# StephenTaf/Modern-Search-Engines-Project

Measured on AMD Instinct MI355X. Metric: queries/sec, two-stage retrieval top-100 (BM25 top-1000 + dense full scan + rerank/fuse), higher is better.
Workload: dtype f32 (exact f32 cosines of every returned document; candidates filtered by one pass of f16 products with a measured margin; batches <= 64 queries: f16x2-split products, |err| <= 8e-6) (dense cosine) / f64 (BM25, fuse)

## Files before the change

include/msretr.h:

```cpp
#ifndef MSRETR_H
#define MSRETR_H

#include <stdint.h>

#ifdef __cplusplus
extern "C" {
#endif

#define MSR_ABI_VERSION 15
#define MSR_DIM 768
#define MSR_MAX_K 1024
#define MSR_MAX_QUERY_TERMS 64
#define MSR_RERANK_MAX_CHUNKS 10
#define MSR_TERMSET_SPAN_DOCS 8192
#define MSR_PHRASE_MAX_TERMS 16
#define MSR_PROX_MAX_SPAN 64
#define MSR_SNIPPET_MAX_WEIGHT (1 << 20)
#define MSR_FUZZY_MAX_LEN 32
#define MSR_FUZZY_MAX_WORDS 1024
#define MSR_FUZZY_MAX_LIMIT 16
#define MSR_FUZZY_SPAN_TERMS 1024
#define MSR_FUZZY_WORD_GROUP 16
#define MSR_WILD_MAX_LEN 32
#define MSR_WILD_MAX_PATTERNS 1024
// ... 13 lines not shown

typedef struct msr_config {
    int32_t struct_size;
    int32_t device;
    int32_t dim;
    int32_t max_queries;
    int32_t max_k;
    int32_t rerank_max_docs;
    int32_t scan_layout;
    int32_t scan_variant;
    int32_t flags;
} msr_config;

#define MSR_CFG_NO_ROW_COPY 1
#define MSR_CFG_SINGLE_EMIT 2

typedef struct msr_rerank_params {
    double smoothing;
    double max_boost;
    double max_decay;
    int32_t max_chunks;
    int32_t reserved;
} msr_rerank_params;

int msr_abi_version(void);
int msr_create(const msr_config* cfg, msr_engine** out);
int msr_destroy(msr_engine* e);
const char* msr_last_error(const msr_engine* e);

int msr_bind_postings(msr_engine* e, const int64_t* term_off, int64_t n_terms, const int32_t* post_doc,
// ... 205 lines not shown
```

modern-search-engines-project_amd/_abi.py:

```python
import ctypes as C
import os

HERE = os.path.dirname(os.path.abspath(__file__))
LIB_PATH = os.path.join(HERE, "csrc", "libmsretr.so")

MSR_ABI_VERSION = 15
MSR_CFG_NO_ROW_COPY = 1
MSR_CFG_SINGLE_EMIT = 2
MSR_DIM = 768
MSR_MAX_K = 1024
MSR_MAX_QUERY_TERMS = 64
MSR_RERANK_MAX_CHUNKS = 10
MSR_MERGE_MAX_ENTRIES = 8192
MSR_TERMSET_SPAN_DOCS = 8192
MSR_PHRASE_MAX_TERMS = 16
MSR_PROX_MAX_SPAN = 64
MSR_SNIPPET_MAX_WEIGHT = 1 << 20
MSR_FUZZY_MAX_LEN = 32
MSR_FUZZY_MAX_WORDS = 1024
MSR_FUZZY_MAX_LIMIT = 16
MSR_FUZZY_SPAN_TERMS = 1024
MSR_FUZZY_WORD_GROUP = 16
MSR_WILD_MAX_LEN = 32
MSR_WILD_MAX_PATTERNS = 1024
# ... 146 lines not shown
```

modern-search-engines-project_amd/csrc/msr_engine.hip:

```cpp
#include <hip/hip_runtime.h>
#include <stdarg.h>
#include <stdio.h>
#include <stdlib.h>
#include <string.h>

#include <algorithm>
#include <new>
#include <vector>

#include "../../include/msretr.h"
#include "msr_devmem.h"
#include "msr_internal.h"

struct HipMem {
    static hipError_t alloc(void** p, size_t bytes) { return hipMalloc(p, bytes); }
    static void free(void* p) { (void)hipFree(p); }
};
using Group = DevGroup<HipMem>;

struct msr_engine {
    msr_config cfg;
    char err[512];
    Group mem_engine;
    Group mem_corpus;
// ... 45 lines not shown
    uint64_t* bm_win = nullptr;
    uint64_t* voc_sig = nullptr;
    int32_t* bt_top_doc = nullptr; float* bt_top_score = nullptr; int32_t* bt_top_n = nullptr;
    int32_t* bt_cand_doc = nullptr; float* bt_cand_score = nullptr; int32_t* bt_cand_chunk = nullptr;
    int32_t* bt_cand_n = nullptr;
    int32_t* tile_row = nullptr;
    int n_tiles = 0;
    bool tiles_ok = false;
    GemmF32Index gf{};
    bool gf_ok = false;
    float* gf_inv_pad = nullptr; float* gf_qn = nullptr; void* gf_fb_qimg = nullptr;
    int32_t* gf_gate = nullptr;
    void* gf_emb_tiled = nullptr;
    void* gf_emb_f16 = nullptr;
    int32_t* tile_trow = nullptr;
    void* emb_bf16 = nullptr;
    GemmIndex gemm{};
    bool gemm_ok = false;
    float* gm_qn = nullptr;
    uint32_t* bf_err = nullptr;
    float* bf_margin = nullptr;
    float* bf_ones = nullptr;
    void* bf_row_meta = nullptr;
    DenseIndex dense_bf16{};
    int n_cus = 256;
    int split_pending = 0;
    int row_copy_state = 0;
    int row_image_state = 0;
    int last_dense_width = 0;
    int last_dense_segments = 0;
// ... 52 lines not shown
    e->mem_postings.release();
}
static void drop_bf16(msr_engine* e) {
    e->dense.emb_bf16 = nullptr;
    e->dense_bf16 = DenseIndex{};
    e->gemm = GemmIndex{};
    e->gemm_ok = false;
    e->mem_bf16.release();
}
static void drop_chunks(msr_engine* e) {
    e->have_chunks = false;
    e->split_pending = 0;
    e->dense = DenseIndex{};
    e->gf = GemmF32Index{};
    e->gf_ok = e->tiles_ok = false;
    e->n_tiles = 0;
    e->row_copy_state = e->row_image_state = 0;
    drop_bf16(e);
    e->mem_chunks.release();
}

template <class T>
static int grow(msr_engine* e, Group& group, T** slot, size_t* have, size_t need, const char* what) {
    if (need <= *have && *slot) return MSR_OK;
    group.free_one(slot);
    *have = 0;
    hipError_t herr = group.alloc(slot, need);
    if (herr != hipSuccess) return fail(e, MSR_ERR_NOMEM, "%s (%zu bytes): %s", what, need, hipGetErrorString(herr));
    *have = need;
    return MSR_OK;
}
// ... 44 lines not shown
    *out = nullptr;
    if (cfg->struct_size != (int32_t)sizeof(msr_config))
        return fail(nullptr, MSR_ERR_INVALID, "msr_create: struct_size %d != %zu", cfg->struct_size, sizeof(msr_config));
    if (cfg->dim != MSR_DIM) return fail(nullptr, MSR_ERR_INVALID, "msr_create: dim must be %d", MSR_DIM);
    if (cfg->max_queries < 1 || cfg->max_queries > 4096)
        return fail(nullptr, MSR_ERR_INVALID, "msr_create: max_queries out of range [1, 4096]");
    if (cfg->max_k < 1 || cfg->max_k > MSR_MAX_K)
        return fail(nullptr, MSR_ERR_INVALID, "msr_create: max_k out of range [1, %d]", MSR_MAX_K);
    if (cfg->rerank_max_docs < 0 || cfg->rerank_max_docs > 1024)
        return fail(nullptr, MSR_ERR_INVALID, "msr_create: rerank_max_docs out of range [0, 1024]");
    if (cfg->scan_layout != 0 && cfg->scan_layout != 1)
        return fail(nullptr, MSR_ERR_INVALID, "msr_create: scan_layout must be 0 or 1");
    if (cfg->scan_variant != 0 && cfg->scan_variant != 2 && cfg->scan_variant != 7 && cfg->scan_variant != 14 &&
        cfg->scan_variant != 15)
        return fail(nullptr, MSR_ERR_INVALID, "msr_create: scan_variant must be 0, 2, 7, 14 or 15");
    if (cfg->flags & ~(int32_t)(MSR_CFG_NO_ROW_COPY | MSR_CFG_SINGLE_EMIT))
        return fail(nullptr, MSR_ERR_INVALID, "msr_create: unknown flag bits 0x%x", cfg->flags);
    int ndev = 0;
    hipError_t herr = hipGetDeviceCount(&ndev);
    if (herr != hipSuccess || ndev <= 0)
        return fail(nullptr, MSR_ERR_HIP, "msr_create: no HIP device available (%s)",
                    herr == hipSuccess ? "device count is 0" : hipGetErrorString(herr));
    if (cfg->device < 0 || cfg->device >= ndev)
        return fail(nullptr, MSR_ERR_INVALID, "msr_create: device %d out of range (have %d)", cfg->device, ndev);
    msr_engine* e = new (std::nothrow) msr_engine();
    if (!e) return fail(nullptr, MSR_ERR_NOMEM, "msr_create: out of host memory");
    e->cfg = *cfg;
    e->err[0] = 0;
    const int rc = create_scratch(e);
    if (rc) {
        fail(nullptr, rc, "msr_create: %s", e->err);
// ... 126 lines not shown
    const Bm25Index cand{term_off, post_doc, post_tf, doc_len, idf, n_terms, n_postings, n_docs, (double)avgdl, k1, b,
                         nullptr, nullptr, (int32_t)((n_docs + MSR_BM25_TILE - 1) / MSR_BM25_TILE), nullptr, nullptr, nullptr, 0};
    const int rc = build_postings(e, cand, (hipStream_t)stream);
    if (rc) drop_postings(e);
    e->have_postings = rc == MSR_OK;
    return rc;
}

struct ChunkLayout {
    std::vector<int32_t> spans, wspans, wspans12;
    int wide_ok = 1, wide_ok64 = 1;
    bool tiles_ok = true;
    std::vector<int32_t> tiles;
    std::vector<int32_t> trow;
    int64_t n_trows = 0;
};

static int chunk_layout(msr_engine* e, int n_cus, const std::vector<int32_t>& h_off, int64_t n_chunks, int64_t n_docs,
                        ChunkLayout& L) {
    if (h_off[0] != 0 || (int64_t)h_off[n_docs] != n_chunks)
        return fail(e, MSR_ERR_INVALID, "msr_bind_chunks: doc_off[0]=%d, doc_off[n_docs]=%d, n_chunks=%lld",
                    h_off[0], h_off[n_docs], (long long)n_chunks);
    for (int64_t d = 0; d < n_docs; ++d)
        if (h_off[d + 1] < h_off[d]) return fail(e, MSR_ERR_INVALID, "msr_bind_chunks: doc_off not monotone at %lld", (long long)d);
    auto make_spans = [&](int target, int64_t min_rows) {
        if ((int64_t)target * min_rows > n_chunks) target = (int)std::max<int64_t>(1, n_chunks / min_rows);
        std::vector<int32_t> sp;
        sp.push_back(0);
        for (int s = 1; s < target; ++s) {
            const int64_t want = n_chunks * s / target;
// ... 47 lines not shown
    L.tiles.push_back(0);
    for (int64_t d = 0; d < n_docs && L.tiles_ok; ++d) {
        const int32_t end = h_off[d + 1];
        if (end - h_off[d] > 256) L.tiles_ok = false;
        if (end - start > 256) { L.tiles.push_back(h_off[d]); start = h_off[d]; }
    }
    if (!L.tiles_ok) return MSR_OK;
    if (L.tiles.back() != (int32_t)n_chunks) L.tiles.push_back((int32_t)n_chunks);
    const size_t n_tiles = L.tiles.size() - 1;
    L.trow.resize(n_tiles);
    for (size_t t = 0; t < n_tiles; ++t) {
        L.trow[t] = (int32_t)L.n_trows;
        L.n_trows += (L.tiles[t + 1] - L.tiles[t] + 15) / 16 * 16;
    }
    if (L.n_trows + MSR_STREAM256_TILE_ROWS >= ((int64_t)1 << 31)) { L.trow.clear(); L.n_trows = 0; }
    return MSR_OK;
}

static int bind_chunk_tables(msr_engine* e, const float* emb, int64_t n_chunks, const int32_t* doc_off, int64_t n_docs,
                             const float* inv_norm, const ChunkLayout& L, hipStream_t st) {
    ALLOC(e, e->mem_chunks, e->chunk_doc, (size_t)n_chunks * sizeof(int32_t));
    ALLOC(e, e->mem_chunks, e->span_doc, L.spans.size() * sizeof(int32_t));
    ALLOC(e, e->mem_chunks, e->wspan_doc, L.wspans.size() * sizeof(int32_t));
    HIP_TRY(e, hipMemcpyAsync(e->span_doc, L.spans.data(), L.spans.size() * sizeof(int32_t), hipMemcpyHostToDevice, st));
    HIP_TRY(e, hipMemcpyAsync(e->wspan_doc, L.wspans.data(), L.wspans.size() * sizeof(int32_t), hipMemcpyHostToDevice, st));
    ALLOC(e, e->mem_chunks, e->wspan12_doc, L.wspans12.size() * sizeof(int32_t));
    HIP_TRY(e, hipMemcpyAsync(e->wspan12_doc, L.wspans12.data(), L.wspans12.size() * sizeof(int32_t), hipMemcpyHostToDevice, st));
    HIP_TRY(e, msr_fill_chunk_doc(doc_off, n_docs, e->chunk_doc, st));
    if (!inv_norm) {
        ALLOC(e, e->mem_chunks, e->inv_norm_own, (size_t)n_chunks * sizeof(float));
// ... 22 lines not shown
        } else {
            ALLOC(e, e->mem_chunks, e->emb_presplit, (size_t)n_chunks * MSR_DIM * sizeof(float));
            HIP_TRY(e, msr_presplit_rows(emb, n_chunks, e->emb_presplit, st));
        }
    }
    e->dense = DenseIndex{emb, doc_off, e->chunk_doc, inv_norm, e->span_doc, n_chunks, n_docs, (n_docs + 31) / 32 * 32,
                          (int)L.spans.size() - 1, e->cfg.scan_layout, e->wspan_doc, (int)L.wspans.size() - 1, e->wspan12_doc,
                          (int)L.wspans12.size() - 1, e->qimg, nullptr, e->emb_presplit, e->row_meta, L.wide_ok,
                          L.wide_ok && L.wide_ok64, nullptr, variant};
    if (L.tiles_ok) {
        ALLOC(e, e->mem_chunks, e->tile_row, L.tiles.size() * 4);
        HIP_TRY(e, hipMemcpyAsync(e->tile_row, L.tiles.data(), L.tiles.size() * 4, hipMemcpyHostToDevice, st));
        e->n_tiles = (int)L.tiles.size() - 1;
        e->tiles_ok = true;
    }
    if (!L.trow.empty()) {
        ALLOC(e, e->mem_chunks, e->tile_trow, L.trow.size() * 4);
        HIP_TRY(e, hipMemcpyAsync(e->tile_trow, L.trow.data(), L.trow.size() * 4, hipMemcpyHostToDevice, st));
    }
    HIP_TRY(e, hipStreamSynchronize(st));
    return MSR_OK;
}

static int bind_stream_pass(msr_engine* e, const ChunkLayout& L, hipStream_t st) {
    if (!(e->tiles_ok && e->dense.variant == 14 && e->n_tiles >= 64)) return MSR_OK;
    const float* emb = e->dense.emb;
    const float* inv_norm = e->dense.inv_norm;
    const int64_t n_chunks = e->dense.n_chunks;
    const int n_tiles = e->n_tiles, nw = e->n_cus * 8, stride = (n_tiles + 31) / 32 * 32;
    const int groups = std::min(8, std::max(e->cfg.max_queries, 128) / 128);
    const int GF_WV_CAP = 4096 * std::max(1, groups / 2);
    const size_t QM = (size_t)groups * 128;
    const int max_nt = std::max(1, std::min(4, groups / 2));
    GemmF32Index& g = e->gf;
    g.n_tiles = n_tiles; g.n_cus = e->n_cus; g.max_groups = groups; g.tmax_stride = stride; g.wv_cap = GF_WV_CAP; g.max_nt = max_nt;
    g.single_emit = (e->cfg.flags & MSR_CFG_SINGLE_EMIT) ? 1 : 0;
    ALLOC(e, e->mem_chunks, e->gf_inv_pad, (size_t)(n_chunks + 512) * 4);
    ALLOC(e, e->mem_chunks, g.qimg, (size_t)groups * 24 * 8192);
    ALLOC(e, e->mem_chunks, e->gf_qn, (QM + 64) * MSR_DIM * 4);
    ALLOC(e, e->mem_chunks, e->gf_fb_qimg, (QM + 63) / 64 * msr_ksplit_slice_image_bytes());
    ALLOC(e, e->mem_chunks, g.tmax_t, (size_t)n_tiles * 8 * (groups >= 2 ? 256 * max_nt : 128) * 4);
    ALLOC(e, e->mem_chunks, g.tmax, QM * stride * 4);
    ALLOC(e, e->mem_chunks, g.thr, QM * 4);
    ALLOC(e, e->mem_chunks, g.thr2, QM * 4);
    ALLOC(e, e->mem_chunks, g.flag, QM * 4);
    ALLOC(e, e->mem_chunks, g.wvbuf, (size_t)nw * GF_WV_CAP * 16);
    ALLOC(e, e->mem_chunks, g.wv_count, (size_t)nw * 4);
    ALLOC(e, e->mem_chunks, g.pairs, QM * 4096 * 8);
    ALLOC(e, e->mem_chunks, g.pair_n, QM * 4);
    ALLOC(e, e->mem_chunks, e->gf_gate, GF_GATE_BYTES);
    ALLOC(e, e->mem_chunks, g.err_max, 4);
    ALLOC(e, e->mem_chunks, g.margin, QM * 4);
    ALLOC(e, e->mem_chunks, g.cand_doc, QM * MSR_SEL_CAP * 4);
    ALLOC(e, e->mem_chunks, g.cand_score, QM * MSR_SEL_CAP * 4);
    ALLOC(e, e->mem_chunks, g.cand_chunk, QM * MSR_SEL_CAP * 4);
    ALLOC(e, e->mem_chunks, g.cand_n, QM * 4);
    g.tile_row = e->tile_row;
    g.inv_pad = e->gf_inv_pad;
    HIP_TRY(e, msr_pad_inv_norm(inv_norm, n_chunks, n_chunks + 512, e->gf_inv_pad, st));
    HIP_TRY(e, hipMemsetAsync(g.pair_n, 0, QM * 4, st));
    HIP_TRY(e, hipMemsetAsync(e->gf_gate, 0, GF_GATE_BYTES, st));
    HIP_TRY(e, hipMemsetAsync(g.cand_n, 0, QM * 4, st));
    HIP_TRY(e, msr_f16_row_error(emb, inv_norm, n_chunks, g.err_max, st));
    if (groups >= 2 && e->tile_trow) {
        const size_t copy_rows = (size_t)L.n_trows + MSR_STREAM256_TILE_ROWS;
        if ((int64_t)L.trow.back() + MSR_STREAM256_TILE_ROWS > (int64_t)copy_rows)
            return fail(e, MSR_ERR_INVALID, "msr_bind_chunks: internal: tile table exceeds the fragment-order copy");
        if (e->cfg.flags & MSR_CFG_NO_ROW_COPY) {
            e->row_copy_state = 2;
        } else if (e->mem_chunks.alloc(&e->gf_emb_tiled, copy_rows * MSR_DIM * 4) != hipSuccess) {
            (void)hipGetLastError();
            e->row_copy_state = 3;
        } else {
            HIP_TRY(e, hipMemsetAsync((char*)e->gf_emb_tiled + (size_t)L.n_trows * MSR_DIM * 4, 0,
                                      (size_t)MSR_STREAM256_TILE_ROWS * MSR_DIM * 4, st));
            HIP_TRY(e, msr_tile_rows(emb, e->tile_row, e->tile_trow, n_tiles, e->gf_emb_tiled, st));
            e->row_copy_state = 1;
        }
    }
    if (max_nt >= 2 && (e->cfg.flags & MSR_CFG_NO_ROW_COPY)) {
        e->row_image_state = 2;
    } else if (max_nt >= 2) {
        const size_t img_rows = (size_t)n_chunks + 512;
        if (e->mem_chunks.alloc(&e->gf_emb_f16, img_rows * MSR_DIM * 2) != hipSuccess) {
            (void)hipGetLastError();
            e->row_image_state = 3;
        } else {
            HIP_TRY(e, msr_f16_rows(emb, n_chunks, (int64_t)img_rows, e->gf_emb_f16, st));
            e->row_image_state = 1;
        }
    }
    g.emb_tiled = e->gf_emb_tiled;
    g.tile_trow = e->gf_emb_tiled ? e->tile_trow : nullptr;
    g.emb_f16 = e->gf_emb_f16;
    e->gf_ok = true;
    return MSR_OK;
}

extern "C" int msr_bind_chunks(msr_engine* e, const float* emb, int64_t n_chunks, const int32_t* doc_off,
                               int64_t n_docs, const float* inv_norm, void* stream) {
    if (!e) return MSR_ERR_INVALID;
    if (!emb || !doc_off || n_chunks <= 0 || n_chunks >= (1ll << 31) || n_docs <= 0 || n_docs >= (1ll << 31))
        return fail(e, MSR_ERR_INVALID, "msr_bind_chunks: bad argument");
    if (e->have_postings && e->bm25.n_docs != n_docs)
        return fail(e, MSR_ERR_INVALID, "msr_bind_chunks: n_docs %lld differs from bound postings (%lld)",
                    (long long)n_docs, (long long)e->bm25.n_docs);
    if (e->cfg.scan_layout == 1 && !inv_norm)
        return fail(e, MSR_ERR_INVALID, "msr_bind_chunks: inv_norm is required with the interleaved layout");
// ... 649 lines not shown
    HIP_TRY(e, msr_dense_scan_slices(ix, e->gf_qn, nq, (float*)e->score_rows, e->gf_fb_qimg, st));
    SelScratch sel = e->sel;
    sel.gate = e->gf_gate; sel.gate_per64 = 1;
    HIP_TRY(e, msr_select_topk(32, e->score_rows, N, e->dense.score_stride, nq, k, sel, out_doc, out_score, out_n, st));
    ix.gate = e->gf_gate; ix.gate_per64 = 1;
    if (out_chunk) HIP_TRY(e, msr_best_chunk(ix, e->gf_qn, nq, k, 0, out_doc, out_n, out_chunk, st));
    return MSR_OK;
}

static bool dense_sweep_wide(const msr_engine* e, int max_chunks_per_doc) {
    return (e->dense.variant == 2 || e->dense.variant == 14 || e->dense.variant == 15) && e->dense.layout == 0 &&
           e->dense.wide_ok && max_chunks_per_doc == 0;
}

static bool dense_stream_ok(const msr_engine* e, int k) {
    return dense_sweep_wide(e, 0) && e->gf_ok && e->dense.variant == 14 && e->gf.n_tiles >= 2 * k;
}

static int dense_stream_cap(const msr_engine* e) { return e->gf.max_groups >= 2 ? (e->gf.max_groups & ~1) * 128 : 128; }

static hipEvent_t* pass_events(msr_engine* e, int kind, hipEvent_t ev[4]) {
    if (!e->timing || e->ev_count[kind] >= msr_engine::EV_RING || e->ev_count[3] >= msr_engine::EV_RING) return nullptr;
    ev[0] = e->ev_start[3][e->ev_count[3]]; ev[1] = e->ev_stop[3][e->ev_count[3]];
    ev[2] = e->ev_start[kind][e->ev_count[kind]]; ev[3] = e->ev_stop[kind][e->ev_count[kind]];
    return ev;
}
static void pass_events_used(msr_engine* e, int kind, const hipEvent_t* ev) {
    if (ev) { e->ev_count[kind]++; e->ev_count[3]++; }
}

extern "C" int msr_dense_split_max(const msr_engine* e, int32_t k) {
// ... 585 lines not shown
```

modern-search-engines-project_amd/csrc/msr_gemm_f32.hip:

```cpp
#include <cmath>
#include <type_traits>

#include "msr_common.h"
#include "msr_internal.h"
#include "msr_frag.h"
#include "msr_gemm_dev.h"

namespace {

constexpr int GF_THREADS = 512;
constexpr int GF_KT = MSR_DIM / 32;
constexpr int GF_ROWB = MSR_DIM * 4;
constexpr int GF_PAIR_CAP = 4096;

typedef StreamArgs GemmF32Args;

__device__ __forceinline__ const char* uniform_ptr(const char* p) {
    const uint64_t u = (uint64_t)p;
    const uint32_t lo = __builtin_amdgcn_readfirstlane((uint32_t)u), hi = __builtin_amdgcn_readfirstlane((uint32_t)(u >> 32));
    return (const char*)(((uint64_t)hi << 32) | lo);
}

constexpr int GS_NB = 8;
constexpr int GS_STEP = 8192;
// ... 322 lines not shown
            return b;
        };
#pragma unroll
        for (int j = 0; j < NNI / 2; ++j) {
            const float lo = a.thr[grp * 256 + (2 * j) * 16 + li16], hi = a.thr[grp * 256 + (2 * j + 1) * 16 + li16];
            thr_h[j] = down_h(lo) | (down_h(hi) << 16);
        }
    }
    constexpr bool JOIN = BF16;
    uint32_t* tmx = (uint32_t*)(smem + G2_TMX);
    if (JOIN) tmx[tid] = 0u;
    auto flush_tmax = [&](int tile_j, int par) {
        const int ln = (int)fresh_lane();
        if (ln < 32) {
            uint32_t* slot = tmx + par * 256 + w * 32 + ln;
            a.tmax_t[(size_t)tile_j * nq_pad + grp * 256 + w * 32 + ln] = ord_val(*slot);
            *slot = 0u;
        }
    };
    float* inv_lds = (float*)(smem + 2 * G2_BLK + 1024) + w * 64;
    auto stage_b = [&](int blk, int pb) {
        const char* base = uniform_ptr(qimg + (size_t)blk * G2_BLK + (size_t)w * 8192);
#pragma unroll
        for (int i = 0; i < 8; ++i)
            __builtin_amdgcn_global_load_lds((glb_void*)(base + (uint32_t)(i * 1024 + lane * 16)),
                                             (lds_void*)(smem + pb * G2_BLK + w * 8192 + i * 1024), 16, 0, 0);
    };
    f32x4 acc[NMI][NNI];
#pragma unroll
    for (int mi = 0; mi < NMI; ++mi)
#pragma unroll
        for (int ni = 0; ni < NNI; ++ni) acc[mi][ni] = (f32x4){0.f, 0.f, 0.f, 0.f};

    auto tile_of = [&](int j) { return a.t_first + j * a.t_stride; };
    auto tile_base = [&](int row0) { return uniform_u64((uint64_t)a.E + (uint64_t)row0 * ROWB); };
    constexpr int NV = (BF16 || TILED) ? 1 : NMI;
    auto row_off = [&](int row0, int mi) -> uint32_t {
        if (TILED) return (uint32_t)(lane * 16);
        if (BF16) return (uint32_t)((WROWS * wr + li16) * ROWB + lg * 32);
        int64_t r = (int64_t)row0 + WROWS * wr + 16 * mi + li16;
        if (r > a.n_rows - 1) r = a.n_rows - 1;
        return (uint32_t)((r - row0) * ROWB + lg * 32);
    };
    int jt = gid;
    int row0 = a.tile_row[tile_of(jt)], row_end = a.tile_row[tile_of(jt) + 1];
    int jn = jt + G < a.t_count ? jt + G : jt;
    int row0n = a.tile_row[tile_of(jn)];
    uint64_t bp = tile_base(TILED ? a.tile_trow[tile_of(jt)] : row0), bn = tile_base(TILED ? a.tile_trow[tile_of(jn)] : row0n);
    uint32_t vp[NV], vn[NV];
#pragma unroll
    for (int mi = 0; mi < NV; ++mi) { vp[mi] = row_off(row0, mi); vn[mi] = row_off(row0n, mi); }

    static_assert(NMI == 2, "the wait counts below assume 4 row loads per ring slot");
    f32x4 ring[RSLOTS][NMI][2];
    auto load_rows = [&](auto slot_c, uint64_t sb, const uint32_t* v, auto off_c) {
        constexpr int slot = decltype(slot_c)::value, off = decltype(off_c)::value;
#pragma unroll
        for (int mi = 0; mi < NMI; ++mi) {
            if (TILED) {
                const uint64_t b = sb + (uint64_t)((2 * wr + mi) * ((GF_KT / KPS) * 2048) + slot * 2048);
                gload16s<0, NTL>(ring[slot][mi][0], v[0], b);
                gload16s<1024, NTL>(ring[slot][mi][1], v[0], b);
            } else {
// ... 144 lines not shown
            if (!(a.dbg & 131072))
#endif
            wg_barrier();
            pb ^= 1;
            if (JOIN && kb == 0 && it > 0) flush_tmax(jt_prev, (it - 1) & 1);
        }
        const int ln_e = (int)fresh_lane();
        const int lg_e = ln_e >> 4;
        f32x4 inv4[NMI];
        if (!BF16 || F16I) {
            if (F16I) asm volatile("s_waitcnt vmcnt(8)" ::: "memory");
            else asm volatile("s_waitcnt vmcnt(12)" ::: "memory");
#pragma unroll
            for (int mi = 0; mi < NMI; ++mi) inv4[mi] = *(const f32x4*)(inv_lds + mi * 16 + 4 * lg_e);
        }
        const int n_valid = row_end - row0;
        const int col_e = wc * 128 + (ln_e & 15);
        float thr_nx = (EMIT && !THR_REGS) ? thr_lds[col_e] : 0.f;
#ifdef MSR_DIAG
        if (a.dbg & 65536) {
#pragma unroll
            for (int ni = 0; ni < NNI; ++ni)
#pragma unroll
                for (int mi = 0; mi < NMI; ++mi) acc[mi][ni] = (f32x4){0.f, 0.f, 0.f, 0.f};
        } else
#endif
#pragma unroll
        for (int ni = 0; ni < NNI; ++ni) {
            f32x4 v[NMI];
            float cmax = NEG_INF;
            const float thr_cur = thr_nx;
// ... 29 lines not shown
                                const int pos = wave_cnt + (int)__builtin_amdgcn_mbcnt_hi((uint32_t)(hm >> 32), __builtin_amdgcn_mbcnt_lo((uint32_t)hm, 0u));
                                if (hit && pos < a.wv_cap)
                                    wvbuf[pos] = make_int4(row0 + rb + rr, q, __float_as_int(x), tile_of(jt));
                                wave_cnt += __popcll(hm);
                            }
                        }
                    }
                }
            }
            float m = cmax;
            auto s32 = __builtin_amdgcn_permlane32_swap(__float_as_uint(m), __float_as_uint(m), false, false);
            m = max2_raw(__uint_as_float(s32[0]), __uint_as_float(s32[1]));
            auto s16 = __builtin_amdgcn_permlane16_swap(__float_as_uint(m), __float_as_uint(m), false, false);
            m = max2_raw(__uint_as_float(s16[0]), __uint_as_float(s16[1]));
            if (JOIN) {
                if (lg_e == 0) atomicMax(tmx + (it & 1) * 256 + ni * 16 + col_e, ord_key(m));
            } else {
                if (lg_e == 0) a.tmax_t[((size_t)jt * 8 + w) * nq_pad + grp * 256 + ni * 16 + col_e] = m;
            }
        }
        jt_prev = jt;
        jt = jn;
        row0 = row0n;
        row_end = a.tile_row[tile_of(jt) + 1];
        jn = jt + G < a.t_count ? jt + G : jt;
        row0n = a.tile_row[tile_of(jn)];
        bp = bn; bn = tile_base(TILED ? a.tile_trow[tile_of(jn)] : row0n);
#pragma unroll
        for (int mi = 0; mi < NV; ++mi) { vp[mi] = vn[mi]; vn[mi] = row_off(row0n, mi); }
    }
    wait_vm0();
    if (JOIN) {
        wg_barrier();
        flush_tmax(jt_prev, (n_mine - 1) & 1);
    }
    if (EMIT && lane == 0) a.wv_count[blockIdx.x * 8 + w] = wave_cnt;
}

template <bool BF16, bool TOBF16 = BF16>
__global__ __launch_bounds__(256) void build_qimg2_kernel(const float* __restrict__ qn, int nq, f16x8* __restrict__ qimg) {
    const int i = blockIdx.x * 256 + threadIdx.x;
    if (i >= GF_KT * 256 * 4) return;
// ... 295 lines not shown
    if (dbg & 8388608) t1 = 2 * t1;
#endif
    if (t1 >= std::max(grid, 2 * k) && T - t1 >= grid) {
        p.n_seg = 2; p.bound[1] = (int)t1; p.bound[2] = T;
    }
    return p;
}

}

hipError_t msr_gemm_f32_pass(const GemmF32Index& g, const DenseIndex& ix, const float* qn, int nq, int k, int k_part,
                             float* out_part, hipEvent_t* ev, int* width_out, int* seg_out, hipStream_t stream) {
    const int W = nq > 128 ? 256 : 128;
    const int waves = 8;
    const int G = (nq + W - 1) / W;
    if (nq <= 0 || G * W > 128 * g.max_groups || k < 1 || g.n_tiles < 2 * k) return hipErrorInvalidValue;
    if (width_out) *width_out = W;
    hipError_t err;
    int NT0 = 1;
    if (W == 256 && (g.n_cus & 7) == 0) NT0 = std::min(std::min(G, g.max_nt), g.n_cus >> 3);
    bool image16 = W == 256 && NT0 > 1 && g.emb_f16 != nullptr;
#ifdef MSR_DIAG
    if (g_f32_dbg & (2048 | 1048576)) image16 = false;
#endif
    if (image16) build_qimg2_kernel<true, false><<<dim3((GF_KT * 256 * 4 + 255) / 256, G), 256, 0, stream>>>(qn, nq, (f16x8*)g.qimg);
    else if (W == 256) build_qimg2_kernel<false><<<dim3((GF_KT * 256 * 4 + 255) / 256, G), 256, 0, stream>>>(qn, nq, (f16x8*)g.qimg);
    else build_qimg1_kernel<<<dim3((GF_KT * 128 * 4 + 255) / 256, G), 256, 0, stream>>>(qn, nq, (f16x8*)g.qimg);
    f16_margin_kernel<<<(nq + 3) / 4, 256, 0, stream>>>(qn, nq, g.err_max, g.margin);
    const float* margin = g.margin;
    const int grid = g.n_cus;
    const PassShape shape = pass_shape(g.n_tiles, k, grid, g.single_emit != 0, g_f32_dbg);
    const int ss = shape.ss, n_s = shape.n_s;
    if (seg_out) *seg_out = shape.n_seg;
    const size_t qimg_bytes = (size_t)GF_KT * W * 64;
    int NT = 1;
    if (W == 256 && (grid & 7) == 0) NT = std::min(std::min(G, g.max_nt), grid >> 3);
#ifdef MSR_DIAG
    if (g_f32_dbg & 2048) NT = 1;
    if (g_f32_dbg & 4096) NT = std::min(NT, 2);
#endif
    GemmF32Args a{};
    a.dbg = g_f32_dbg; a.nt = 1;
    a.E = (const char*)ix.emb; a.inv_pad = g.inv_pad; a.tile_row = g.tile_row;
    bool tiled = W == 256 && g.emb_tiled != nullptr && !image16;
#ifdef MSR_DIAG
    if (g_f32_dbg & 8192) tiled = false;
#endif
    if (tiled) { a.E = (const char*)g.emb_tiled; a.tile_trow = g.tile_trow; }
    if (image16) a.E = (const char*)g.emb_f16;
    const int tmax_parts = image16 ? 1 : waves;
    a.n_rows = ix.n_chunks; a.tmax_t = g.tmax_t;
    a.t_first = ss / 2; a.t_stride = ss; a.t_count = n_s;
    for (int gi = 0; gi < G; gi += NT) {
        a.nt = std::min(NT, G - gi);
        a.qimg = (const char*)g.qimg + gi * qimg_bytes;
        if (ev && gi == 0 && (err = hipEventRecord(ev[0], stream)) != hipSuccess) return err;
        if ((err = launch_f32(W, false, a, grid, stream, tiled, image16)) != hipSuccess) return err;
        if (ev && gi == 0 && (err = hipEventRecord(ev[1], stream)) != hipSuccess) return err;
// ... 6 lines not shown
        const int t0 = shape.bound[s], t1 = shape.bound[s + 1];
        a.t_first = t0; a.t_count = t1 - t0;
        for (int gi = 0; gi < G; gi += NT) {
            a.nt = std::min(NT, G - gi);
            a.qimg = (const char*)g.qimg + gi * qimg_bytes;
            a.thr = g.thr + gi * W; a.q_base = gi * W; a.append = (s > 0 || gi > 0);
            if (ev && gi == 0 && s == 0 && (err = hipEventRecord(ev[2], stream)) != hipSuccess) return err;
            if ((err = launch_f32(W, true, a, grid, stream, tiled, image16)) != hipSuccess) return err;
            if (ev && gi == 0 && s == shape.n_seg - 1 && (err = hipEventRecord(ev[3], stream)) != hipSuccess) return err;
            if ((err = msr_gemm_tmax(g.tmax_t, t1 - t0, tmax_parts, W * a.nt, g.tmax + (size_t)gi * W * g.tmax_stride + t0, g.tmax_stride, stream)) != hipSuccess) return err;
        }
        if (s + 1 < shape.n_seg &&
            (err = msr_gemm_kth(g.tmax, t1, g.tmax_stride, nq, W * G, k, margin, g.thr, nullptr, stream, __builtin_inff(), 1.0f, true)) != hipSuccess)
            return err;
    }
    if ((err = msr_gemm_kth(g.tmax, g.n_tiles, g.tmax_stride, nq, W * G, k, margin, g.thr2, nullptr, stream)) != hipSuccess) return err;
    if (out_part && (err = msr_gemm_kth(g.tmax, g.n_tiles, g.tmax_stride, nq, nq, k_part, margin, out_part, nullptr, stream,
                                        -__builtin_inff(), 0.5f)) != hipSuccess) return err;
    return hipSuccess;
}

namespace {
__global__ __launch_bounds__(256) void raise_thr_kernel(float* __restrict__ thr2, const float* __restrict__ bound,
                                                         const float* __restrict__ margin, int nq) {
    const int q = blockIdx.x * 256 + threadIdx.x;
    if (q >= nq) return;
    const float b = bound[q] - 0.5f * margin[q];
    if (b > thr2[q]) thr2[q] = b;
}
}

hipError_t msr_gemm_f32_finish(const GemmF32Index& g, const DenseIndex& ix, const float* qn, int nq, int k, const float* bound,
// ... 26 lines not shown
```

modern-search-engines-project_amd/csrc/msr_internal.h:

```cpp
#pragma once
#include <hip/hip_runtime.h>
#include <stdint.h>

#define MSR_DIM 768
#define MSR_SEL_BINS 4096
#define MSR_SEL_CAP 4096

struct SelState {
    uint64_t pref_hi, mask_hi;
    uint32_t pref_lo, mask_lo;
    int32_t k_rem;
    int32_t n_above;
    int32_t done;
    int32_t n_sel;
};

struct SelScratch {
    uint32_t* hist;
    SelState* state;
    uint64_t* cand_hi;
    uint32_t* cand_lo;
    int32_t* cand_n;
    const int32_t* gate;
    int gate_per64;
// ... 274 lines not shown
hipError_t msr_unit_bf16_rows(const float* src, const float* inv_norm, int64_t n_rows, int64_t n_pad, void* dst,
                              uint32_t* err_max, hipStream_t stream);
hipError_t msr_batch_margin(const float* qn, int nq, const uint32_t* err_max, float* margin, hipStream_t stream);
hipError_t msr_gemm_candidates(const GemmIndex& g, const DenseIndex& ix, const float* qn, int nq, int k, const float* margin,
                               int32_t* cand_doc, int32_t* cand_first_len, int32_t* cand_n, hipEvent_t* ev,
                               hipStream_t stream);

constexpr int MSR_STREAM256_TILE_ROWS = 256;

struct StreamArgs {
    const char* E;
    const float* inv_pad;
    const char* qimg;
    const int32_t* tile_row;
    const int32_t* tile_trow;
    int64_t n_rows;
    int t_first, t_stride, t_count;
    float* tmax_t;
    const float* thr;
    void* wvbuf; int wv_cap; int32_t* wv_count;
    int q_base;
    int append;
    int nt;
    int dbg;
};
hipError_t msr_stream256_bf16_launch(bool emit, const StreamArgs& a, int grid, hipStream_t stream);
hipError_t msr_stream256_bf16_qimage(const float* qn, int nq, int n_groups, void* qimg, hipStream_t stream);

struct GemmF32Index {
    const int32_t* tile_row;
    int32_t n_tiles;
    int32_t n_cus;
    int32_t max_groups;
    const float* inv_pad;
    void* qimg;
    float* tmax_t;
    float* tmax;
    int32_t tmax_stride;
    float* thr; float* thr2; int32_t* flag;
    void* wvbuf; int32_t wv_cap; int32_t* wv_count;
    void* pairs; int32_t* pair_n;
    uint32_t* err_max; float* margin;
    int32_t* cand_doc; float* cand_score; int32_t* cand_chunk; int32_t* cand_n;
    int32_t max_nt;
    const void* emb_tiled;
    const int32_t* tile_trow;
// ... 26 lines not shown
```

modern-search-engines-project_amd/engine.py:

```python
import ctypes as C

import numpy as np
import torch

from . import _abi
from .index import DIM, CorpusIndex

RERANK_DEFAULTS = dict(smoothing=0.15, max_boost=0.1, max_decay=0.05, max_chunks=10)


def _ptr(t):
    return C.c_void_p(t.data_ptr()) if t is not None else C.c_void_p(0)


STREAM_MIN_BYTES = 64 << 20
_NP_OF = {torch.float32: np.float32, torch.float64: np.float64, torch.int32: np.int32, torch.int64: np.int64,
          torch.int16: np.int16}


def stream_to_device(arr, device, block_bytes=128 << 20):
    dev = torch.device(device)
    out = torch.empty(arr.shape, dtype=torch.from_numpy(np.empty(0, arr.dtype)).dtype, device=dev)
    if arr.size == 0:
        return out
# ... 9 lines not shown
        if done[b & 1] is not None:
            done[b & 1].synchronize()
        n = (r1 - r0) * row
        np.copyto(buf.numpy()[:n].reshape((r1 - r0,) + tuple(arr.shape[1:])), arr[r0:r1])
        flat_out[r0 * row:r0 * row + n].copy_(buf[:n], non_blocking=pinned)
        if pinned:
            done[b & 1] = torch.cuda.Event()
            done[b & 1].record(torch.cuda.current_stream(dev))
    if pinned:
        torch.cuda.current_stream(dev).synchronize()
    return out


class DeviceEngine:
    def __init__(self, index: CorpusIndex, device=0, max_queries=32, max_k=1000, rerank_max_docs=1000,
                 scan_layout=0, scan_variant=0, row_copy=True, single_emit=False):
        if not torch.cuda.is_available():
            raise _abi.MsrError(-102, "no GPU visible: the retrieval path runs on MI355X only (no CPU fallback)")
        self.lib = _abi.load()
        self.index = index
        self.device = torch.device("cuda", device) if isinstance(device, int) else torch.device(device)
        self.max_k = int(max_k)
        self.max_queries = int(max_queries)
        self.scan_layout = int(scan_layout)
        self.rerank_max_docs = int(rerank_max_docs)
        cfg = _abi.MsrConfig(C.sizeof(_abi.MsrConfig), self.device.index or 0, DIM, int(max_queries), int(max_k),
                             int(rerank_max_docs), int(scan_layout), int(scan_variant),
                             (0 if row_copy else _abi.MSR_CFG_NO_ROW_COPY) | (_abi.MSR_CFG_SINGLE_EMIT if single_emit else 0))
        self.handle = C.c_void_p()
        rc = self.lib.msr_create(C.byref(cfg), C.byref(self.handle))
        if rc != 0:
            raise _abi.MsrError(rc, (self.lib.msr_last_error(None) or b"?").decode())
        self._t = {}
        self._bf16 = False
        self._bind(index)

    def _stream(self):
        return C.c_void_p(torch.cuda.current_stream(self.device).cuda_stream)

    def _dev(self, x, dtype):
        if x is None:
            return None
        if torch.is_tensor(x):
# ... 863 lines not shown
```

Measured before the change: 59930.

## Use fixed 256-row tiles for the wide dense scan instead of document-aligned tiles

By default, the wide (256-query) f32 dense scan now tiles the chunk matrix into fixed 256-row tiles rather than document-aligned tiles. Each tile carries a head count of rows that belong to a document started in the previous tile, and the per-tile maximum is dropped for waves covering only those rows. This removes the padding rows that document-aligned tiles add and gives uniform tile sizes, so the row-copy image is smaller and work is better balanced. In exchange it adds head bookkeeping, empty-tile -inf handling and a separate tile count for the kth-threshold pass, and the old layout is kept behind a new DOC_TILES flag.

```diff
diff --git a/include/msretr.h b/include/msretr.h
--- a/include/msretr.h
+++ b/include/msretr.h
@@ -51,6 +51,7 @@
 
 #define MSR_CFG_NO_ROW_COPY 1
 #define MSR_CFG_SINGLE_EMIT 2
+#define MSR_CFG_DOC_TILES 4
 
 typedef struct msr_rerank_params {
     double smoothing;
diff --git a/modern-search-engines-project_amd/_abi.py b/modern-search-engines-project_amd/_abi.py
--- a/modern-search-engines-project_amd/_abi.py
+++ b/modern-search-engines-project_amd/_abi.py
@@ -7,6 +7,7 @@
 MSR_ABI_VERSION = 15
 MSR_CFG_NO_ROW_COPY = 1
 MSR_CFG_SINGLE_EMIT = 2
+MSR_CFG_DOC_TILES = 4
 MSR_DIM = 768
 MSR_MAX_K = 1024
 MSR_MAX_QUERY_TERMS = 64
diff --git a/modern-search-engines-project_amd/csrc/msr_engine.hip b/modern-search-engines-project_amd/csrc/msr_engine.hip
--- a/modern-search-engines-project_amd/csrc/msr_engine.hip
+++ b/modern-search-engines-project_amd/csrc/msr_engine.hip
@@ -83,6 +83,9 @@
     void* gf_emb_tiled = nullptr;
     void* gf_emb_f16 = nullptr;
     int32_t* tile_trow = nullptr;
+    int32_t* rtile_row = nullptr;
+    int32_t* rtile_head = nullptr;
+    int n_rtiles = 0;
     void* emb_bf16 = nullptr;
     GemmIndex gemm{};
     bool gemm_ok = false;
@@ -165,7 +168,7 @@
     e->dense = DenseIndex{};
     e->gf = GemmF32Index{};
     e->gf_ok = e->tiles_ok = false;
-    e->n_tiles = 0;
+    e->n_tiles = e->n_rtiles = 0;
     e->row_copy_state = e->row_image_state = 0;
     drop_bf16(e);
     e->mem_chunks.release();
@@ -240,7 +243,7 @@
     if (cfg->scan_variant != 0 && cfg->scan_variant != 2 && cfg->scan_variant != 7 && cfg->scan_variant != 14 &&
         cfg->scan_variant != 15)
         return fail(nullptr, MSR_ERR_INVALID, "msr_create: scan_variant must be 0, 2, 7, 14 or 15");
-    if (cfg->flags & ~(int32_t)(MSR_CFG_NO_ROW_COPY | MSR_CFG_SINGLE_EMIT))
+    if (cfg->flags & ~(int32_t)(MSR_CFG_NO_ROW_COPY | MSR_CFG_SINGLE_EMIT | MSR_CFG_DOC_TILES))
         return fail(nullptr, MSR_ERR_INVALID, "msr_create: unknown flag bits 0x%x", cfg->flags);
     int ndev = 0;
     hipError_t herr = hipGetDeviceCount(&ndev);
@@ -397,6 +400,8 @@
     std::vector<int32_t> tiles;
     std::vector<int32_t> trow;
     int64_t n_trows = 0;
+    std::vector<int32_t> rtiles;
+    std::vector<int32_t> rhead;
 };
 
 static int chunk_layout(msr_engine* e, int n_cus, const std::vector<int32_t>& h_off, int64_t n_chunks, int64_t n_docs,
@@ -474,6 +479,17 @@
         L.n_trows += (L.tiles[t + 1] - L.tiles[t] + 15) / 16 * 16;
     }
     if (L.n_trows + MSR_STREAM256_TILE_ROWS >= ((int64_t)1 << 31)) { L.trow.clear(); L.n_trows = 0; }
+    const int64_t n_rt = (n_chunks + 255) / 256;
+    L.rtiles.resize((size_t)n_rt + 1);
+    L.rhead.resize((size_t)n_rt);
+    int64_t d = 0;
+    for (int64_t t = 0; t < n_rt; ++t) {
+        const int64_t r = 256 * t;
+        L.rtiles[t] = (int32_t)r;
+        while (h_off[d + 1] <= r) ++d;
+        L.rhead[t] = h_off[d] < r ? (int32_t)(std::min<int64_t>(h_off[d + 1], n_chunks) - r) : 0;
+    }
+    L.rtiles[n_rt] = (int32_t)n_chunks;
     return MSR_OK;
 }
 
@@ -526,9 +542,17 @@
         e->n_tiles = (int)L.tiles.size() - 1;
         e->tiles_ok = true;
     }
-    if (!L.trow.empty()) {
-        ALLOC(e, e->mem_chunks, e->tile_trow, L.trow.size() * 4);
-        HIP_TRY(e, hipMemcpyAsync(e->tile_trow, L.trow.data(), L.trow.size() * 4, hipMemcpyHostToDevice, st));
+    if (L.tiles_ok && (e->cfg.flags & MSR_CFG_DOC_TILES)) {
+        if (!L.trow.empty()) {
+            ALLOC(e, e->mem_chunks, e->tile_trow, L.trow.size() * 4);
+            HIP_TRY(e, hipMemcpyAsync(e->tile_trow, L.trow.data(), L.trow.size() * 4, hipMemcpyHostToDevice, st));
+        }
+    } else if (L.tiles_ok) {
+        ALLOC(e, e->mem_chunks, e->rtile_row, L.rtiles.size() * 4);
+        ALLOC(e, e->mem_chunks, e->rtile_head, L.rhead.size() * 4);
+        HIP_TRY(e, hipMemcpyAsync(e->rtile_row, L.rtiles.data(), L.rtiles.size() * 4, hipMemcpyHostToDevice, st));
+        HIP_TRY(e, hipMemcpyAsync(e->rtile_head, L.rhead.data(), L.rhead.size() * 4, hipMemcpyHostToDevice, st));
+        e->n_rtiles = (int)L.rhead.size();
     }
     HIP_TRY(e, hipStreamSynchronize(st));
     return MSR_OK;
@@ -539,19 +563,21 @@
     const float* emb = e->dense.emb;
     const float* inv_norm = e->dense.inv_norm;
     const int64_t n_chunks = e->dense.n_chunks;
-    const int n_tiles = e->n_tiles, nw = e->n_cus * 8, stride = (n_tiles + 31) / 32 * 32;
+    const bool row_tiles = e->rtile_row != nullptr;
+    const int n_tiles = e->n_tiles, n_tiles256 = row_tiles ? e->n_rtiles : n_tiles, nw = e->n_cus * 8;
+    const int max_tiles = std::max(n_tiles, n_tiles256), stride = (max_tiles + 31) / 32 * 32;
     const int groups = std::min(8, std::max(e->cfg.max_queries, 128) / 128);
     const int GF_WV_CAP = 4096 * std::max(1, groups / 2);
     const size_t QM = (size_t)groups * 128;
     const int max_nt = std::max(1, std::min(4, groups / 2));
     GemmF32Index& g = e->gf;
-    g.n_tiles = n_tiles; g.n_cus = e->n_cus; g.max_groups = groups; g.tmax_stride = stride; g.wv_cap = GF_WV_CAP; g.max_nt = max_nt;
+    g.n_tiles = n_tiles; g.n_tiles256 = n_tiles256; g.n_cus = e->n_cus; g.max_groups = groups; g.tmax_stride = stride; g.wv_cap = GF_WV_CAP; g.max_nt = max_nt;
     g.single_emit = (e->cfg.flags & MSR_CFG_SINGLE_EMIT) ? 1 : 0;
     ALLOC(e, e->mem_chunks, e->gf_inv_pad, (size_t)(n_chunks + 512) * 4);
     ALLOC(e, e->mem_chunks, g.qimg, (size_t)groups * 24 * 8192);
     ALLOC(e, e->mem_chunks, e->gf_qn, (QM + 64) * MSR_DIM * 4);
     ALLOC(e, e->mem_chunks, e->gf_fb_qimg, (QM + 63) / 64 * msr_ksplit_slice_image_bytes());
-    ALLOC(e, e->mem_chunks, g.tmax_t, (size_t)n_tiles * 8 * (groups >= 2 ? 256 * max_nt : 128) * 4);
+    ALLOC(e, e->mem_chunks, g.tmax_t, (size_t)max_tiles * 8 * (groups >= 2 ? 256 * max_nt : 128) * 4);
     ALLOC(e, e->mem_chunks, g.tmax, QM * stride * 4);
     ALLOC(e, e->mem_chunks, g.thr, QM * 4);
     ALLOC(e, e->mem_chunks, g.thr2, QM * 4);
@@ -568,15 +594,20 @@
     ALLOC(e, e->mem_chunks, g.cand_chunk, QM * MSR_SEL_CAP * 4);
     ALLOC(e, e->mem_chunks, g.cand_n, QM * 4);
     g.tile_row = e->tile_row;
+    g.tile_row256 = row_tiles ? e->rtile_row : e->tile_row;
+    g.tile_head256 = row_tiles ? e->rtile_head : nullptr;
     g.inv_pad = e->gf_inv_pad;
     HIP_TRY(e, msr_pad_inv_norm(inv_norm, n_chunks, n_chunks + 512, e->gf_inv_pad, st));
     HIP_TRY(e, hipMemsetAsync(g.pair_n, 0, QM * 4, st));
     HIP_TRY(e, hipMemsetAsync(e->gf_gate, 0, GF_GATE_BYTES, st));
     HIP_TRY(e, hipMemsetAsync(g.cand_n, 0, QM * 4, st));
     HIP_TRY(e, msr_f16_row_error(emb, inv_norm, n_chunks, g.err_max, st));
-    if (groups >= 2 && e->tile_trow) {
-        const size_t copy_rows = (size_t)L.n_trows + MSR_STREAM256_TILE_ROWS;
-        if ((int64_t)L.trow.back() + MSR_STREAM256_TILE_ROWS > (int64_t)copy_rows)
+    const int64_t n_trows = row_tiles ? (n_chunks + 15) / 16 * 16 : L.n_trows;
+    const int32_t* copy_trow = row_tiles ? e->rtile_row : e->tile_trow;
+    if (groups >= 2 && copy_trow && n_trows + MSR_STREAM256_TILE_ROWS < ((int64_t)1 << 31)) {
+        const size_t copy_rows = (size_t)n_trows + MSR_STREAM256_TILE_ROWS;
+        const int64_t last_trow = row_tiles ? L.rtiles[L.rtiles.size() - 2] : L.trow.back();
+        if (last_trow + MSR_STREAM256_TILE_ROWS > (int64_t)copy_rows)
             return fail(e, MSR_ERR_INVALID, "msr_bind_chunks: internal: tile table exceeds the fragment-order copy");
         if (e->cfg.flags & MSR_CFG_NO_ROW_COPY) {
             e->row_copy_state = 2;
@@ -584,9 +615,9 @@
             (void)hipGetLastError();
             e->row_copy_state = 3;
         } else {
-            HIP_TRY(e, hipMemsetAsync((char*)e->gf_emb_tiled + (size_t)L.n_trows * MSR_DIM * 4, 0,
+            HIP_TRY(e, hipMemsetAsync((char*)e->gf_emb_tiled + (size_t)n_trows * MSR_DIM * 4, 0,
                                       (size_t)MSR_STREAM256_TILE_ROWS * MSR_DIM * 4, st));
-            HIP_TRY(e, msr_tile_rows(emb, e->tile_row, e->tile_trow, n_tiles, e->gf_emb_tiled, st));
+            HIP_TRY(e, msr_tile_rows(emb, g.tile_row256, copy_trow, n_tiles256, e->gf_emb_tiled, st));
             e->row_copy_state = 1;
         }
     }
@@ -603,7 +634,7 @@
         }
     }
     g.emb_tiled = e->gf_emb_tiled;
-    g.tile_trow = e->gf_emb_tiled ? e->tile_trow : nullptr;
+    g.tile_trow = e->gf_emb_tiled ? copy_trow : nullptr;
     g.emb_f16 = e->gf_emb_f16;
     e->gf_ok = true;
     return MSR_OK;
@@ -1283,7 +1314,7 @@
 }
 
 static bool dense_stream_ok(const msr_engine* e, int k) {
-    return dense_sweep_wide(e, 0) && e->gf_ok && e->dense.variant == 14 && e->gf.n_tiles >= 2 * k;
+    return dense_sweep_wide(e, 0) && e->gf_ok && e->dense.variant == 14 && std::min(e->gf.n_tiles, e->gf.n_tiles256) >= 2 * k;
 }
 
 static int dense_stream_cap(const msr_engine* e) { return e->gf.max_groups >= 2 ? (e->gf.max_groups & ~1) * 128 : 128; }
diff --git a/modern-search-engines-project_amd/csrc/msr_gemm_f32.hip b/modern-search-engines-project_amd/csrc/msr_gemm_f32.hip
--- a/modern-search-engines-project_amd/csrc/msr_gemm_f32.hip
+++ b/modern-search-engines-project_amd/csrc/msr_gemm_f32.hip
@@ -360,7 +360,8 @@
         const int ln = (int)fresh_lane();
         if (ln < 32) {
             uint32_t* slot = tmx + par * 256 + w * 32 + ln;
-            a.tmax_t[(size_t)tile_j * nq_pad + grp * 256 + w * 32 + ln] = ord_val(*slot);
+            const uint32_t u = *slot;
+            a.tmax_t[(size_t)tile_j * nq_pad + grp * 256 + w * 32 + ln] = u ? ord_val(u) : -__builtin_inff();
             *slot = 0u;
         }
     };
@@ -388,11 +389,23 @@
         if (r > a.n_rows - 1) r = a.n_rows - 1;
         return (uint32_t)((r - row0) * ROWB + lg * 32);
     };
+    typedef const __attribute__((address_space(4))) int32_t* ctab;
+    const ctab t_row = (ctab)a.tile_row, t_trow = (ctab)a.tile_trow, t_head = (ctab)a.tile_head;
+    const bool rowt = a.tile_head != nullptr;
+    auto tile_first = [&](int j) -> int { return rowt ? tile_of(j) * MSR_STREAM256_TILE_ROWS : t_row[tile_of(j)]; };
+    auto tile_rows = [&](int j, int first) -> int {
+        if (rowt) {
+            const int64_t left = a.n_rows - first;
+            return (left < MSR_STREAM256_TILE_ROWS ? (int)left : MSR_STREAM256_TILE_ROWS) | (t_head[tile_of(j)] << 16);
+        }
+        return t_row[tile_of(j) + 1] - first;
+    };
+    auto copy_first = [&](int j, int first) -> int { return (TILED && !rowt) ? t_trow[tile_of(j)] : first; };
     int jt = gid;
-    int row0 = a.tile_row[tile_of(jt)], row_end = a.tile_row[tile_of(jt) + 1];
+    int row0 = tile_first(jt), nv_head = tile_rows(jt, row0);
     int jn = jt + G < a.t_count ? jt + G : jt;
-    int row0n = a.tile_row[tile_of(jn)];
-    uint64_t bp = tile_base(TILED ? a.tile_trow[tile_of(jt)] : row0), bn = tile_base(TILED ? a.tile_trow[tile_of(jn)] : row0n);
+    int row0n = tile_first(jn), nv_head_n = tile_rows(jn, row0n);
+    uint64_t bp = tile_base(copy_first(jt, row0)), bn = tile_base(copy_first(jn, row0n));
     uint32_t vp[NV], vn[NV];
 #pragma unroll
     for (int mi = 0; mi < NV; ++mi) { vp[mi] = row_off(row0, mi); vn[mi] = row_off(row0n, mi); }
@@ -567,7 +580,8 @@
 #pragma unroll
             for (int mi = 0; mi < NMI; ++mi) inv4[mi] = *(const f32x4*)(inv_lds + mi * 16 + 4 * lg_e);
         }
-        const int n_valid = row_end - row0;
+        const int n_valid = nv_head & 0xffff;
+        const bool owns = WROWS * wr >= (nv_head >> 16);
         const int col_e = wc * 128 + (ln_e & 15);
         float thr_nx = (EMIT && !THR_REGS) ? thr_lds[col_e] : 0.f;
 #ifdef MSR_DIAG
@@ -627,18 +641,19 @@
             auto s16 = __builtin_amdgcn_permlane16_swap(__float_as_uint(m), __float_as_uint(m), false, false);
             m = max2_raw(__uint_as_float(s16[0]), __uint_as_float(s16[1]));
             if (JOIN) {
-                if (lg_e == 0) atomicMax(tmx + (it & 1) * 256 + ni * 16 + col_e, ord_key(m));
+                if (lg_e == 0 && owns) atomicMax(tmx + (it & 1) * 256 + ni * 16 + col_e, ord_key(m));
             } else {
-                if (lg_e == 0) a.tmax_t[((size_t)jt * 8 + w) * nq_pad + grp * 256 + ni * 16 + col_e] = m;
+                if (lg_e == 0) a.tmax_t[((size_t)jt * 8 + w) * nq_pad + grp * 256 + ni * 16 + col_e] = owns ? m : NEG_INF;
             }
         }
         jt_prev = jt;
         jt = jn;
         row0 = row0n;
-        row_end = a.tile_row[tile_of(jt) + 1];
+        nv_head = nv_head_n;
         jn = jt + G < a.t_count ? jt + G : jt;
-        row0n = a.tile_row[tile_of(jn)];
-        bp = bn; bn = tile_base(TILED ? a.tile_trow[tile_of(jn)] : row0n);
+        row0n = tile_first(jn);
+        nv_head_n = tile_rows(jn, row0n);
+        bp = bn; bn = tile_base(copy_first(jn, row0n));
 #pragma unroll
         for (int mi = 0; mi < NV; ++mi) { vp[mi] = vn[mi]; vn[mi] = row_off(row0n, mi); }
     }
@@ -964,7 +979,8 @@
     const int W = nq > 128 ? 256 : 128;
     const int waves = 8;
     const int G = (nq + W - 1) / W;
-    if (nq <= 0 || G * W > 128 * g.max_groups || k < 1 || g.n_tiles < 2 * k) return hipErrorInvalidValue;
+    const int T = W == 256 ? g.n_tiles256 : g.n_tiles;
+    if (nq <= 0 || G * W > 128 * g.max_groups || k < 1 || T < 2 * k) return hipErrorInvalidValue;
     if (width_out) *width_out = W;
     hipError_t err;
     int NT0 = 1;
@@ -979,7 +995,7 @@
     f16_margin_kernel<<<(nq + 3) / 4, 256, 0, stream>>>(qn, nq, g.err_max, g.margin);
     const float* margin = g.margin;
     const int grid = g.n_cus;
-    const PassShape shape = pass_shape(g.n_tiles, k, grid, g.single_emit != 0, g_f32_dbg);
+    const PassShape shape = pass_shape(T, k, grid, g.single_emit != 0, g_f32_dbg);
     const int ss = shape.ss, n_s = shape.n_s;
     if (seg_out) *seg_out = shape.n_seg;
     const size_t qimg_bytes = (size_t)GF_KT * W * 64;
@@ -991,7 +1007,9 @@
 #endif
     GemmF32Args a{};
     a.dbg = g_f32_dbg; a.nt = 1;
-    a.E = (const char*)ix.emb; a.inv_pad = g.inv_pad; a.tile_row = g.tile_row;
+    a.E = (const char*)ix.emb; a.inv_pad = g.inv_pad;
+    a.tile_row = W == 256 ? g.tile_row256 : g.tile_row;
+    a.tile_head = W == 256 ? g.tile_head256 : nullptr;
     bool tiled = W == 256 && g.emb_tiled != nullptr && !image16;
 #ifdef MSR_DIAG
     if (g_f32_dbg & 8192) tiled = false;
@@ -1028,8 +1046,8 @@
             (err = msr_gemm_kth(g.tmax, t1, g.tmax_stride, nq, W * G, k, margin, g.thr, nullptr, stream, __builtin_inff(), 1.0f, true)) != hipSuccess)
             return err;
     }
-    if ((err = msr_gemm_kth(g.tmax, g.n_tiles, g.tmax_stride, nq, W * G, k, margin, g.thr2, nullptr, stream)) != hipSuccess) return err;
-    if (out_part && (err = msr_gemm_kth(g.tmax, g.n_tiles, g.tmax_stride, nq, nq, k_part, margin, out_part, nullptr, stream,
+    if ((err = msr_gemm_kth(g.tmax, T, g.tmax_stride, nq, W * G, k, margin, g.thr2, nullptr, stream)) != hipSuccess) return err;
+    if (out_part && (err = msr_gemm_kth(g.tmax, T, g.tmax_stride, nq, nq, k_part, margin, out_part, nullptr, stream,
                                         -__builtin_inff(), 0.5f)) != hipSuccess) return err;
     return hipSuccess;
 }
diff --git a/modern-search-engines-project_amd/csrc/msr_internal.h b/modern-search-engines-project_amd/csrc/msr_internal.h
--- a/modern-search-engines-project_amd/csrc/msr_internal.h
+++ b/modern-search-engines-project_amd/csrc/msr_internal.h
@@ -312,6 +312,7 @@
     const char* qimg;
     const int32_t* tile_row;
     const int32_t* tile_trow;
+    const int32_t* tile_head;
     int64_t n_rows;
     int t_first, t_stride, t_count;
     float* tmax_t;
@@ -328,6 +329,9 @@
 struct GemmF32Index {
     const int32_t* tile_row;
     int32_t n_tiles;
+    const int32_t* tile_row256;
+    const int32_t* tile_head256;
+    int32_t n_tiles256;
     int32_t n_cus;
     int32_t max_groups;
     const float* inv_pad;
diff --git a/modern-search-engines-project_amd/engine.py b/modern-search-engines-project_amd/engine.py
--- a/modern-search-engines-project_amd/engine.py
+++ b/modern-search-engines-project_amd/engine.py
@@ -47,7 +47,7 @@
 
 class DeviceEngine:
     def __init__(self, index: CorpusIndex, device=0, max_queries=32, max_k=1000, rerank_max_docs=1000,
-                 scan_layout=0, scan_variant=0, row_copy=True, single_emit=False):
+                 scan_layout=0, scan_variant=0, row_copy=True, single_emit=False, doc_tiles=False):
         if not torch.cuda.is_available():
             raise _abi.MsrError(-102, "no GPU visible: the retrieval path runs on MI355X only (no CPU fallback)")
         self.lib = _abi.load()
@@ -59,7 +59,8 @@
         self.rerank_max_docs = int(rerank_max_docs)
         cfg = _abi.MsrConfig(C.sizeof(_abi.MsrConfig), self.device.index or 0, DIM, int(max_queries), int(max_k),
                              int(rerank_max_docs), int(scan_layout), int(scan_variant),
-                             (0 if row_copy else _abi.MSR_CFG_NO_ROW_COPY) | (_abi.MSR_CFG_SINGLE_EMIT if single_emit else 0))
+                             (0 if row_copy else _abi.MSR_CFG_NO_ROW_COPY) | (_abi.MSR_CFG_SINGLE_EMIT if single_emit else 0) |
+                             (_abi.MSR_CFG_DOC_TILES if doc_tiles else 0))
         self.handle = C.c_void_p()
         rc = self.lib.msr_create(C.byref(cfg), C.byref(self.handle))
         if rc != 0:
```

After: 59990 (median of 6 runs). About the same (+0.1%).
